# reuk/parallel-reverb-raytracer

Hardware: AMD Instinct MI355X
Metric: ray_bounces_per_sec (higher is better)
Workload: dtype f32; 1 GPU; cathedral stand-in (Sibenik unavailable offline), 75252 triangles, 100000 rays/GPU x 128 bounces x 8 bands, 2 cardioid speakers, 44100 Hz, trim_predelay, output_mode all, histogram mode exact; triangles=75252, rays_per_gpu=100000, reflections=128, histogram_mode=exact: the reference's serial float sum over all impulses, bit for bit

## Files before the change

include/rvb_capi.h:

```cpp
#ifndef RVB_CAPI_H
#define RVB_CAPI_H

#include <stdint.h>

#ifdef __cplusplus
extern "C" {
#endif

#define RVB_NUM_IMAGE_SOURCE 10
#define RVB_NUM_BANDS 8

enum {
    RVB_OK = 0,
    RVB_ERR_INVALID = 1,
    RVB_ERR_NO_DEVICE = 2,
    RVB_ERR_HIP = 3,
    RVB_ERR_STATE = 4,
    RVB_ERR_CAPACITY = 5
};

typedef struct { uint64_t surface, v0, v1, v2; } rvb_triangle;
typedef struct { float s[4]; } rvb_float3;
typedef struct { float specular[8]; float diffuse[8]; } rvb_surface;
typedef struct { float volume[8]; float position[4]; float time; float pad_[3]; } rvb_impulse;
// ... 17 lines not shown
int rvb_record_event(rvb_ctx * ctx, void * hip_event);
int rvb_device_info(rvb_ctx * ctx, char * arch, uint64_t arch_capacity, int * compute_units, uint64_t * hbm_bytes);
int rvb_device_index(rvb_ctx * ctx, int * device);

int rvb_set_scene(rvb_ctx * ctx,
                  const rvb_triangle * triangles, uint64_t ntriangles,
                  const rvb_float3 * vertices, uint64_t nvertices,
                  const rvb_surface * surfaces, uint64_t nsurfaces);
int rvb_share_scene(rvb_ctx * ctx, rvb_ctx * from);
int rvb_scene_info(rvb_ctx * ctx, uint64_t * nodes, uint64_t * kept_triangles, uint32_t * depth);

int rvb_set_directions(rvb_ctx * ctx, const rvb_float3 * directions, uint64_t nrays);
int rvb_set_directions_device(rvb_ctx * ctx, const void * d_directions, uint64_t nrays);
int rvb_set_concurrent_traces(rvb_ctx * ctx, uint32_t traces);
int rvb_set_path_lanes(rvb_ctx * ctx, uint32_t lanes);

int rvb_trace(rvb_ctx * ctx, const float mic[3], const float source[3],
              uint64_t nreflections, const float air_coefficient[8], uint64_t ray_offset);

int rvb_trace_pairs(rvb_ctx * ctx, const float * mics, const float * sources, uint64_t npairs,
                    uint64_t nreflections, const float air_coefficient[8], uint64_t ray_offset);

int rvb_trace_group(rvb_ctx ** ctxs, uint64_t count, const float * mics, const float * sources, uint64_t nreflections,
                    const float air_coefficient[8], const uint64_t * ray_offsets);
typedef struct { float direction[4]; float shape[8]; } rvb_source_pattern;
int rvb_set_source_pattern(rvb_ctx * ctx, const rvb_source_pattern * patterns, uint64_t npatterns);

int rvb_keep_paths(rvb_ctx * ctx, int keep);
int rvb_reshade(rvb_ctx * ctx, const rvb_surface * surfaces, uint64_t nsurfaces, const float air_coefficient[8]);

// ... 122 lines not shown
```

parallel-reverb-raytracer_amd/capi.py:

```python
import ctypes
import os

import numpy as np

from .dtypes import ATTENUATED, IMPULSE, SPEAKER, SURFACE, aligned_zeros

_HERE = os.path.dirname(os.path.abspath(__file__))
LIB_PATH = os.environ.get("RVB_LIB", os.path.join(_HERE, "librvb_hip.so"))

IMAGE_CANDIDATE = np.dtype([("ray", "<u8"), ("slot", "<u4"), ("index", "<u4"), ("impulse", IMPULSE)])
assert IMAGE_CANDIDATE.itemsize == 80

IR_DIFFUSE, IR_IMAGES, IR_ALL = 1, 2, 3
IR_FAST, IR_EXACT = 0, 1

SYMBOLS = [
    "rvb_create", "rvb_destroy", "rvb_last_error", "rvb_synchronize", "rvb_wait_for_event", "rvb_device_info",
    "rvb_set_scene", "rvb_share_scene", "rvb_scene_info", "rvb_set_directions", "rvb_set_directions_device", "rvb_set_concurrent_traces", "rvb_set_path_lanes", "rvb_trace", "rvb_trace_group",
    "rvb_trace_pairs", "rvb_ir_select_pair",
    "rvb_get_diffuse", "rvb_diffuse_device", "rvb_get_direct", "rvb_get_image_candidates", "rvb_merge_images",
    "rvb_attenuate_speaker", "rvb_attenuate_speaker_device", "rvb_attenuate_hrtf", "rvb_attenuate_hrtf_device", "rvb_flatten",
    "rvb_ir_configure_speakers", "rvb_ir_configure_hrtf", "rvb_ir_time_range", "rvb_ir_time_range_begin", "rvb_ir_bins", "rvb_ir_accumulate", "rvb_ir_accumulate_export", "rvb_ir_exact_prepare", "rvb_ir_exact_fold", "rvb_record_event",
    "rvb_ir_download", "rvb_last_timings", "rvb_debug_stamps", "rvb_executed_bounces",
    "rvb_device_alloc", "rvb_device_free", "rvb_copy_to_host", "rvb_copy_to_device", "rvb_fix_predelay_device", "rvb_flatten_device",
    "rvb_host_alloc", "rvb_host_free", "rvb_copy_to_pinned_host_async", "rvb_synchronize_exports",
    "rvb_multi_create", "rvb_multi_destroy", "rvb_multi_last_error", "rvb_multi_devices", "rvb_multi_context", "rvb_multi_used_rccl", "rvb_multi_set_chain_blocks", "rvb_multi_peer_links",
    "rvb_multi_set_scene", "rvb_multi_set_directions", "rvb_multi_trace", "rvb_multi_get_diffuse", "rvb_multi_get_images",
    "rvb_multi_ir_speakers", "rvb_multi_ir_hrtf",
    "rvb_device_index", "rvb_pipeline_create", "rvb_pipeline_destroy", "rvb_pipeline_last_error", "rvb_pipeline_configure_speakers",
    "rvb_pipeline_configure_hrtf", "rvb_pipeline_submit", "rvb_pipeline_submit_oriented", "rvb_pipeline_pending", "rvb_pipeline_next",
    "rvb_pipeline_create_lanes",
    "rvb_set_source_pattern", "rvb_multi_set_source_pattern", "rvb_pipeline_set_source_pattern", "rvb_pipeline_submit_directed",
    "rvb_keep_paths", "rvb_reshade",
# ... 174 lines not shown
        handles = (ctypes.c_void_p * n)(*[c.handle for c in contexts])
        m = np.ascontiguousarray(np.asarray(mics, dtype=np.float32).reshape(n, 3))
        s = np.ascontiguousarray(np.asarray(sources, dtype=np.float32).reshape(n, 3))
        offs = (ctypes.c_uint64 * n)(*[int(o) for o in (ray_offsets if ray_offsets is not None else [0] * n)])
        contexts[0]._check(contexts[0].lib.rvb_trace_group(handles, _u64(n), _ptr(m), _ptr(s), _u64(nreflections), _f8(air), offs))
        for c in contexts:
            c.nreflections = int(nreflections)
            c.npairs = 1

    def set_concurrent_traces(self, traces):
        self._check(self.lib.rvb_set_concurrent_traces(self.handle, ctypes.c_uint32(int(traces))))

    def set_path_lanes(self, lanes):
        self._check(self.lib.rvb_set_path_lanes(self.handle, ctypes.c_uint32(int(lanes))))

    def set_source_pattern(self, direction, shape=None):
        if direction is None or shape is None:
            self._check(self.lib.rvb_set_source_pattern(self.handle, None, _u64(0)))
            return
        pats = make_source_patterns(direction, shape)
        self._check(self.lib.rvb_set_source_pattern(self.handle, pats, _u64(len(pats))))

    def keep_paths(self, on):
        self._check(self.lib.rvb_keep_paths(self.handle, ctypes.c_int(1 if on else 0)))

    def reshade(self, surfaces, air):
        table, count = surface_table(surfaces)
        self._check(self.lib.rvb_reshade(self.handle, _ptr(table), _u64(count), _f8(air)))

    def trace(self, mic, source, nreflections, air, ray_offset=0):
# ... 383 lines not shown
```

parallel-reverb-raytracer_amd/csrc/bvh.h:

```cpp
#pragma once

#include <stdint.h>
#include <string>
#include <vector>

#include "../../include/rvb_capi.h"

#define RVB_BVH_EMPTY 0xFFFFFFFFu
#define RVB_BVH_LEAF 0x80000000u
#define RVB_BVH_NODE_SHIFT 6
#ifndef RVB_BVH_MAX_LEAF
#define RVB_BVH_MAX_LEAF 4
#endif
#define RVB_BVH_STACK 64

struct BvhChild {
    uint16_t lox, hix, loy, hiy, loz, hiz;
    uint32_t ref;
};
struct BvhNode { BvhChild c[4]; };

struct BvhTri {
    float v0[3];
    float e0[3];
    float e1[3];
    uint32_t index;
    uint32_t surface;
    uint32_t pad;
};

struct TriCorners { float v[9]; float pad[3]; };

struct TriShade { float n[3]; uint32_t surface; uint32_t skip_ref; float skip_a; float skip_b; uint32_t group; };

struct BuiltScene {
    std::vector<BvhNode> nodes;
    std::vector<BvhTri> tris;
    std::vector<TriShade> shade;
    std::vector<TriCorners> corners;
    std::vector<uint32_t> leafpos;
    uint32_t depth = 0;
    uint32_t stack_need = 0;
    float pad = 0.0f;
    float bounds_lo[3] = {0, 0, 0}, bounds_hi[3] = {0, 0, 0};
};

std::string rvb_build_scene(const rvb_triangle * triangles, uint64_t ntriangles,
                            const rvb_float3 * vertices, uint64_t nvertices,
                            uint64_t nsurfaces, BuiltScene & out);
```

parallel-reverb-raytracer_amd/csrc/bvh_build.hip:

```cpp
#include "bvh.h"
#include "rvb_math.h"

#include <algorithm>
#include <cmath>
#include <cstdlib>
#include <cstring>
#include <limits>
#include <queue>
#include <tuple>

namespace {

struct Box {
    float lo[3], hi[3];
    void reset()
    {
        for (int a = 0; a < 3; ++a) { lo[a] = std::numeric_limits<float>::infinity(); hi[a] = -lo[a]; }
    }
    void grow(const float p[3])
    {
        for (int a = 0; a < 3; ++a) { lo[a] = std::min(lo[a], p[a]); hi[a] = std::max(hi[a], p[a]); }
    }
    void grow(const Box & b)
    {
// ... 360 lines not shown
        TriShade & sk = out.shade[t.index];
        sk.group = gid[t.index];
        if (sk.skip_ref == RVB_BVH_EMPTY) continue;
        const PlaneGroup & pg = pl.groups[gid[t.index]];
        const TriGeo & g = pl.geo[t.index];
        const double A = 6.0 * pg.delta + pg.g + 32.0 * eps * g.kappa * g.L + 1.74 * eps * (double) maxabs;
        const double B = 16.0 * eps * g.kappa + 4.0 * eps;
        const double C = 2.0 * pg.theta + pg.d + 8.0 * eps;
        const double a = std::max(0.01, C + A * (1.0 + 1e-4) / EPS), b = B * (1.0 + 1e-4) / EPS;
        sk.skip_a = std::nextafterf((float) a, 2.0f);
        sk.skip_b = std::nextafterf((float) b, 2.0f);
        if (!(a < 1.0)) sk.skip_ref = RVB_BVH_EMPTY;
    }
}

}

std::string rvb_build_scene(const rvb_triangle * triangles, uint64_t ntriangles,
                            const rvb_float3 * vertices, uint64_t nvertices,
                            uint64_t nsurfaces, BuiltScene & out)
{
    if (ntriangles >= (1ull << 24))
        return "too many triangles (limit 2^24: triangle byte offsets are formed with a 24-bit multiply, node references are 31-bit byte offsets)";
    out = BuiltScene();
    out.shade.resize(ntriangles);
    out.corners.resize(ntriangles);

    float maxabs = 0.0f;
    Box scene;
    scene.reset();
// ... 181 lines not shown
    for (size_t i = out.nodes.size(); i-- > 0;) {
        uint32_t nchild = 0, deepest = 0;
        for (int k = 0; k < 4; ++k) {
            uint32_t c = out.nodes[i].c[k].ref;
            if (c == RVB_BVH_EMPTY)
                continue;
            ++nchild;
            if (!(c & RVB_BVH_LEAF))
                deepest = std::max(deepest, need[c >> RVB_BVH_NODE_SHIFT]);
        }
        need[i] = (nchild ? nchild - 1 : 0) + deepest;
    }
    out.stack_need = need[0] + 1;
    if (out.stack_need <= RVB_BVH_STACK) {
        assign_skips(out, planes, maxabs);
        return "";
    }
    }
    return "BVH needs a deeper traversal stack than " + std::to_string(RVB_BVH_STACK) + " entries";
}
```

parallel-reverb-raytracer_amd/csrc/context.hip:

```cpp
#include "ctx.h"

#include <cstring>

static thread_local std::string g_create_error;

int fail(rvb_ctx * ctx, int code, const std::string & what)
{
    if (ctx) ctx->error = what; else g_create_error = what;
    return code;
}

extern "C" {

int rvb_create(rvb_ctx ** out, int device, unsigned flags)
{
    (void) flags;
    if (!out)
        return fail(nullptr, RVB_ERR_INVALID, "rvb_create: out is NULL");
    *out = nullptr;
    int count = 0;
    hipError_t e = hipGetDeviceCount(&count);
    if (e != hipSuccess || count <= 0)
        return fail(nullptr, RVB_ERR_NO_DEVICE,
                    std::string("rvb_create: no HIP device (") + (e != hipSuccess ? hipGetErrorString(e) : "count 0") +
// ... 104 lines not shown
        ctx->store = std::make_shared<SceneStore>();
        ctx->store->device = ctx->device;
    }
    SceneStore & st = *ctx->store;
    auto upload = [&](DevBuf & b, const void * src, size_t bytes) -> hipError_t {
        hipError_t e = b.ensure(bytes);
        if (e != hipSuccess || bytes == 0) return e;
        return hipMemcpy(b.p, src, bytes, hipMemcpyHostToDevice);
    };
    RVB_HIP(fail, ctx, upload(st.nodes, built.nodes.data(), built.nodes.size() * sizeof(BvhNode)));
    RVB_HIP(fail, ctx, upload(st.tris, built.tris.data(), built.tris.size() * sizeof(BvhTri)));
    for (size_t i = 0; i < built.shade.size() && i < built.leafpos.size(); ++i) built.shade[i].group = built.leafpos[i];
    RVB_HIP(fail, ctx, upload(st.shade, built.shade.data(), built.shade.size() * sizeof(TriShade)));
    RVB_HIP(fail, ctx, upload(st.corners, built.corners.data(), built.corners.size() * sizeof(TriCorners)));
    RVB_HIP(fail, ctx, upload(st.surfaces, surfaces, nsurfaces * sizeof(rvb_surface)));
    ctx->scene.nodes = st.nodes.as<const BvhNode>();
    ctx->scene.tris = st.tris.as<const BvhTri>();
    ctx->scene.shade = st.shade.as<const TriShade>();
    ctx->scene.corners = st.corners.as<const TriCorners>();
    ctx->scene.surfaces = st.surfaces.as<const rvb_surface>();
    ctx->scene.ntris = (uint32_t) built.tris.size();
    ctx->scene.cull_abs = built.pad;
    ctx->scene.cull_rel = 1e-4f;
    ctx->nnodes = built.nodes.size();
    ctx->kept = built.tris.size();
    ctx->depth = built.depth;
    ctx->stack_need = built.stack_need;
    ctx->nsurfaces = nsurfaces;
    ctx->have_scene = true;
    return RVB_OK;
// ... 2 lines not shown
int rvb_share_scene(rvb_ctx * ctx, rvb_ctx * from)
{
    if (!ctx || !from) return RVB_ERR_INVALID;
    if (ctx == from) return RVB_OK;
    if (!from->have_scene || !from->store) return fail(ctx, RVB_ERR_STATE, "rvb_share_scene: the other context holds no scene");
    if (from->device != ctx->device) return fail(ctx, RVB_ERR_INVALID, "rvb_share_scene: the contexts are on different devices (a scene is shared within one GPU's memory)");
    RVB_BIND(ctx);
    RVB_HIP(fail, ctx, hipStreamSynchronize(ctx->stream));
    ctx->store = from->store;
    ctx->scene = from->scene;
    ctx->nnodes = from->nnodes;
    ctx->kept = from->kept;
    ctx->depth = from->depth;
    ctx->stack_need = from->stack_need;
    ctx->nsurfaces = from->nsurfaces;
    ctx->have_scene = true;
    ctx->traced = false;
    return RVB_OK;
}

int rvb_scene_info(rvb_ctx * ctx, uint64_t * nodes, uint64_t * kept_triangles, uint32_t * depth)
{
    if (!ctx) return RVB_ERR_INVALID;
    if (!ctx->have_scene) return fail(ctx, RVB_ERR_STATE, "rvb_scene_info: no scene");
    if (nodes) *nodes = ctx->nnodes;
    if (kept_triangles) *kept_triangles = ctx->kept;
    if (depth) *depth = ctx->depth;
    return RVB_OK;
}

// ... 30 lines not shown
}

int rvb_set_concurrent_traces(rvb_ctx * ctx, uint32_t traces)
{
    if (!ctx) return RVB_ERR_INVALID;
    if (traces == 0 || traces > (1u << 20)) return fail(ctx, RVB_ERR_INVALID, "rvb_set_concurrent_traces: 1 .. 2^20");
    ctx->concurrent_traces = traces;
    return RVB_OK;
}

int rvb_set_path_lanes(rvb_ctx * ctx, uint32_t lanes)
{
    if (!ctx) return RVB_ERR_INVALID;
    if (lanes != 0 && lanes != 1 && lanes != 2 && lanes != 4) return fail(ctx, RVB_ERR_INVALID, "rvb_set_path_lanes: 0 (automatic), 1, 2 or 4");
    ctx->path_lanes = lanes;
    return RVB_OK;
}

int rvb_last_timings(rvb_ctx * ctx, char * names, uint64_t names_capacity, float * ms, uint64_t ms_capacity, uint64_t * count)
{
    if (!ctx || !count) return RVB_ERR_INVALID;
    RVB_BIND(ctx);
    RVB_HIP(fail, ctx, hipStreamSynchronize(ctx->stream));
    std::string joined;
    uint64_t n = 0;
    for (const Timing & t : ctx->timings) {
        float v = 0.0f;
        RVB_HIP(fail, ctx, hipEventElapsedTime(&v, t.start, t.stop));
        if (ms && n < ms_capacity) ms[n] = v;
        if (!joined.empty()) joined += ';';
// ... 36 lines not shown
```

parallel-reverb-raytracer_amd/csrc/ctx.h:

```cpp
#pragma once

#include "../../include/rvb_capi.h"
#include "hip_owned.h"
#include "kernels.h"

#include <cmath>
#include <cstddef>
#include <memory>
#include <string>
#include <vector>

#pragma GCC visibility push(hidden)

struct SceneStore {
    int device = 0;
    DevBuf nodes, tris, shade, corners, surfaces;
    ~SceneStore() { (void) hipSetDevice(device); }
};

struct SmallBlock {
    uint32_t candidate_count;
    uint32_t pad0_;
    unsigned long long executed;
    uint32_t range[2];
    uint32_t max_time_bits;
    uint32_t pad1_;
    uint32_t trace_range[2];
    uint32_t image_item_count;
    uint32_t pad2_[5];
    rvb_impulse direct;
};
// ... 13 lines not shown
    Event export_ready;
    Event path_done, side_done;
    Event prep_done, group_done;
    std::string error;
    std::string arch;
    int compute_units = 0;
    uint64_t hbm_bytes = 0;

    bool have_scene = false;
    std::shared_ptr<SceneStore> store;
    SceneDev scene;
    uint64_t nnodes = 0, kept = 0;
    uint32_t depth = 0;
    uint32_t stack_need = RVB_BVH_STACK;
    uint64_t nsurfaces = 0;

    DevBuf directions_own;
    const float4 * directions = nullptr;
    uint64_t nrays = 0;
    uint32_t concurrent_traces = 1;
    uint32_t path_lanes = 0;
    bool range_pending = false;
    int hrtf_table_ears = 0;
    bool traced = false;
    uint64_t nreflections = 0;
    float mic[3] = {0, 0, 0};
    uint64_t npairs = 1, traced_rays = 0, ir_pair = 0;
    std::vector<float> pair_mics_host;
    DevBuf pair_geom, pair_direct, pair_range;
    PinnedBuf pair_stage;
// ... 111 lines not shown
```

parallel-reverb-raytracer_amd/csrc/kernels.h:

```cpp
#pragma once

#include <hip/hip_runtime.h>
#include <stdint.h>

#include "../../include/rvb_capi.h"
#include "bvh.h"

struct SceneDev {
    const BvhNode * nodes = nullptr;
    const BvhTri * tris = nullptr;
    const TriShade * shade = nullptr;
    const TriCorners * corners = nullptr;
    const rvb_surface * surfaces = nullptr;
    uint32_t ntris = 0;
    float cull_abs = 0.0f;
    float cull_rel = 0.0f;
    unsigned long long * stamps = nullptr;
};

struct ImageItem { uint32_t ray, index; };
struct TraceArgs {
    SceneDev scene;
    const float4 * directions;
    rvb_impulse * impulses;
// ... 12 lines not shown
    uint32_t * time_range;
    uint64_t nrays;
    uint32_t nreflections;
    uint32_t stack_entries;
    uint32_t lds_surfaces;
    uint32_t path_lanes;
    uint32_t npairs;
    uint32_t rays_per_pair;
    const float4 * pair_mics;
    const float4 * pair_sources;
    uint64_t ray_offset;
    float mic[3];
    float source[3];
    float air[8];
    float * image_dist;
};

void rvb_launch_path(const TraceArgs & a, hipStream_t s);
uint32_t rvb_lds_surfaces(uint32_t stack_entries, uint64_t nsurfaces);
uint32_t rvb_path_lanes_for(uint64_t nrays, uint32_t concurrent);
#define RVB_MAX_GROUP 4
void rvb_launch_path_group(const TraceArgs * traces, uint32_t count, hipStream_t s);
uint32_t rvb_shadow_lanes();
void rvb_launch_images(const TraceArgs & a, hipStream_t s);
void rvb_launch_shadow(const TraceArgs & a, hipStream_t s);
struct SourcePatternDev { float direction[4]; float shape[8]; };
SourcePatternDev rvb_source_pattern_device_form(const rvb_source_pattern & p);
void rvb_launch_source_pattern(const TraceArgs & a, const SourcePatternDev * patterns, uint32_t npatterns, hipStream_t s);
void rvb_launch_path_keep(const TraceArgs & a, float4 * kept, hipStream_t s);
uint32_t rvb_reshade_lds_surfaces(uint64_t nsurfaces);
void rvb_launch_reshade(const TraceArgs & a, const float4 * kept, hipStream_t s);
void rvb_launch_reshade_images(const TraceArgs & a, hipStream_t s);
size_t rvb_group_records_temp_bytes(uint64_t n);
hipError_t rvb_group_records(void * temp, size_t temp_bytes, const uint32_t * keys, uint32_t * keys_scratch, uint32_t * order,
                             uint64_t n, uint32_t first_record, int begin_bit, int end_bit, hipStream_t s);
hipError_t rvb_group_records16(void * temp, size_t temp_bytes, const uint16_t * keys, uint16_t * keys_scratch, uint32_t * order,
                               uint64_t n, uint32_t first_record, int begin_bit, int end_bit, hipStream_t s);

#define RVB_HRTF_ROWS (360 * 180 + 1)
struct AttenuationModel {
// ... 45 lines not shown
```

parallel-reverb-raytracer_amd/csrc/shadow_kernels.hip:

```cpp
#include "traversal.h"

#include <algorithm>
#include <cstdlib>

namespace {

template <bool SURF_LDS>
struct ShadowJob {
    const TraceArgs & a;
    uint32_t c;
    uint64_t g, stride, total;
    v3 mic;
    float airA, airB;
    float4 * rec;
    float4 mine;
    v3 p;
    float diff, new_dist, mag;
    uint32_t surface;
    float tmin, tmax_seen;
    uint32_t pair;
    lds_float4_ptr surf_lds;
    uint32_t skip;

    __device__ __forceinline__ uint32_t skip_ref() const { return skip; }
// ... 112 lines not shown
            const float4 m4 = a.pair_mics[tag - 1u];
            mic = mk3(m4.x, m4.y, m4.z);
            pair = tag - 1u;
        }
        const float new_dist = dpp_f<QP_PAIR_HI>(aux.x), threshold = dpp_f<QP_PAIR_HI>(aux.y);
        const float4 * shade = reinterpret_cast<const float4 *>(a.scene.shade + dpp_u<QP_PAIR_HI>(__float_as_uint(aux.z)));
        const float4 sh = shade[0];
        const uint32_t skip_ref = __float_as_uint(shade[1].x);
        const uint32_t surface = __float_as_uint(sh.w);
        const v3 p = mk3(dpp_f<QP_PAIR_LO>(aux.x), dpp_f<QP_PAIR_LO>(aux.y), dpp_f<QP_PAIR_LO>(aux.z));
        const float diff = dpp_f<QP_PAIR_LO>(aux.w);
        const v3 b2p = mic - p;
        const float mag = length3(b2p);
        const v3 dir = normalize3(b2p);
        const uint32_t skip = fabsf(dot3(mk3(sh.x, sh.y, sh.z), dir)) > threshold ? skip_ref : RVB_BVH_EMPTY;
        const bool visible = !traverse_pair_any(a.scene, p, dir, mag, stack, skip);
        const float dist = visible ? new_dist + mag : 0.0f;
        float4 o = make_float4(0, 0, 0, 0);
        if (visible) {
            const float4 dc = surface_row<SURF_LDS>(a, surf_lds, surface, 2 + h);
            o.x = band_product(vol.x, air_attenuation(dist, air0) * 1.0f, dc.x, diff);
            o.y = band_product(vol.y, air_attenuation(dist, air1) * 1.0f, dc.y, diff);
            o.z = band_product(vol.z, air_attenuation(dist, air2) * 1.0f, dc.z, diff);
            o.w = band_product(vol.w, air_attenuation(dist, air3) * 1.0f, dc.w, diff);
        }
        const float t = seconds_per_meter() * dist;
        store_stream(rec + h, o);
        store_stream(rec + h + 2, h == 0 ? make_float4(p.x, p.y, p.z, 0.0f) : make_float4(t, 0.0f, 0.0f, 0.0f));
        uint32_t nonzero = (o.x != 0.0f || o.y != 0.0f || o.z != 0.0f || o.w != 0.0f) ? 1u : 0u;
        nonzero |= dpp_u<QP_SWAP1>(nonzero);
        if (nonzero) {
// ... 114 lines not shown
            o_hi.z = band_product(vol_hi.z, air_attenuation(dist, a.air[6]) * 1.0f, d_hi.z, diff);
            o_hi.w = band_product(vol_hi.w, air_attenuation(dist, a.air[7]) * 1.0f, d_hi.w, diff);
        }
        const float t = seconds_per_meter() * dist;
        store_stream(rec + 0, o_lo);
        store_stream(rec + 1, o_hi);
        store_stream(rec + 2, make_float4(p.x, p.y, p.z, 0.0f));
        store_stream(rec + 3, make_float4(t, 0.0f, 0.0f, 0.0f));
        const bool nonzero = o_lo.x != 0.0f || o_lo.y != 0.0f || o_lo.z != 0.0f || o_lo.w != 0.0f
                          || o_hi.x != 0.0f || o_hi.y != 0.0f || o_hi.z != 0.0f || o_hi.w != 0.0f;
        note_time(a, nonzero, true, pair, t, tmin, tmax_seen);
    }
    time_range_of_wave(a, tmin, tmax_seen);
}

}

uint32_t rvb_shadow_lanes()
{
    static const int lanes = getenv("RVB_SHADOW_LANES") ? atoi(getenv("RVB_SHADOW_LANES")) : 2;
    return lanes == 4 ? 4u : (lanes == 1 ? 1u : 2u);
}

void rvb_launch_shadow(const TraceArgs & a, hipStream_t s)
{
    const uint64_t total = a.nrays * (uint64_t) a.nreflections;
    if (total == 0) return;
    static const char * const per_cu_env = getenv("RVB_SHADOW_WG_PER_CU");
    static const uint64_t per_cu_set = per_cu_env ? strtoull(per_cu_env, nullptr, 10) : 0;
    const uint32_t lanes = rvb_shadow_lanes();
// ... 10 lines not shown
```

parallel-reverb-raytracer_amd/csrc/trace.hip:

```cpp
#include "ctx.h"

#include <algorithm>
#include <cstdlib>
#include <cstring>
#include <map>

namespace {

struct TracePlan {
    TraceArgs a;
    uint64_t npairs = 1, nrays = 0, nreflections = 0;
    int key_bits = 1;
};

int upload_source_patterns(rvb_ctx * ctx)
{
    if (ctx->source_dirty && !ctx->source_patterns.empty()) {
        const size_t bytes = ctx->source_patterns.size() * sizeof(SourcePatternDev);
        if (bytes > ctx->source_stage.cap || bytes > ctx->source_dev.cap) {
            if (ctx->source_dev.p) RVB_HIP(fail, ctx, hipStreamSynchronize(ctx->stream));
            RVB_HIP(fail, ctx, ctx->source_stage.ensure(bytes));
            RVB_HIP(fail, ctx, ctx->source_dev.ensure(bytes));
        }
        if (!ctx->source_stage_free) RVB_HIP(fail, ctx, hipEventCreateWithFlags(&ctx->source_stage_free.h, hipEventDisableTiming));
// ... 68 lines not shown
    a.impulses = ctx->impulses.as<rvb_impulse>();
    a.early = ctx->early.as<uint32_t>();
    a.candidates = ctx->candidates.as<rvb_image_candidate>();
    a.candidate_count = &small->candidate_count;
    a.image_items = reinterpret_cast<ImageItem *>(ctx->image_items.p);
    a.image_state = ctx->image_items.as<uint32_t>() + ((size_t) nrays * 9 + npairs) * 2;
    a.image_item_count = &small->image_item_count;
    a.direct = &small->direct;
    a.npairs = (uint32_t) npairs;
    a.rays_per_pair = (uint32_t) ctx->nrays;
    a.pair_mics = nullptr;
    a.pair_sources = nullptr;
    a.executed = &small->executed;
    a.time_range = small->trace_range;
    a.image_dist = ctx->keep_paths ? ctx->kept_image_dist.as<float>() : nullptr;
    if (npairs > 1) {
        const size_t geom_floats = 8 * npairs, init_words = 2 * npairs;
        const size_t stage_bytes = geom_floats * sizeof(float) + init_words * sizeof(uint32_t);
        if (stage_bytes > ctx->pair_stage.cap) {
            if (ctx->pair_stage.p) RVB_HIP(fail, ctx, hipStreamSynchronize(ctx->stream));
            RVB_HIP(fail, ctx, ctx->pair_stage.ensure(stage_bytes));
        }
        if (!ctx->pair_stage_free) RVB_HIP(fail, ctx, hipEventCreateWithFlags(&ctx->pair_stage_free.h, hipEventDisableTiming));
        else RVB_HIP(fail, ctx, hipEventSynchronize(ctx->pair_stage_free));
        float * geom = ctx->pair_stage.as<float>();
        uint32_t * init = reinterpret_cast<uint32_t *>(geom + geom_floats);
        std::memset(geom, 0, geom_floats * sizeof(float));
        for (uint64_t p = 0; p < npairs; ++p)
            for (int i = 0; i < 3; ++i) { geom[4 * p + i] = mics[3 * p + i]; geom[4 * (npairs + p) + i] = sources[3 * p + i]; }
        for (uint64_t p = 0; p < npairs; ++p) { init[2 * p] = 0xFFFFFFFFu; init[2 * p + 1] = 0u; }
// ... 60 lines not shown
    TraceArgs & a = plan.a;
    const uint64_t npairs = plan.npairs, nrays = plan.nrays, nreflections = plan.nreflections;
    const int key_bits = plan.key_bits;
    static const int group_bits = getenv("RVB_SHADOW_SORT_BITS") ? atoi(getenv("RVB_SHADOW_SORT_BITS")) : 16;
    RVB_HIP(fail, ctx, hipEventRecord(ctx->path_done, ctx->stream));
    RVB_HIP(fail, ctx, hipStreamWaitEvent(ctx->side_stream, ctx->path_done, 0));
    ctx->begin_timing("image_kernel", ctx->side_stream);
    a.scene.stamps = nullptr;
    rvb_launch_images(a, ctx->side_stream);
    ctx->end_timing(ctx->side_stream);
    RVB_HIP(fail, ctx, hipEventRecord(ctx->side_done, ctx->side_stream));
    a.scene.stamps = ctx->stamps.as<unsigned long long>() + 16;
    if (ctx->keep_paths) {
        ctx->begin_timing("path_keep_kernel");
        rvb_launch_path_keep(a, ctx->kept_paths.as<float4>(), ctx->stream);
        ctx->end_timing();
        RVB_HIP(fail, ctx, hipGetLastError());
    }
    if (a.sort_keys || a.sort_keys16) {
        ctx->begin_timing("record_sort_kernels");
        a.sort_order = ctx->sort_order.as<uint32_t>();
        RVB_HIP(fail, ctx, hipGetLastError());
        const uint64_t per_pair = ctx->nrays * nreflections;
        for (uint64_t p = 0; p < npairs; ++p) {
            if (a.sort_keys16) {
                const int end = std::min(16, key_bits);
                RVB_HIP(fail, ctx, rvb_group_records16(ctx->group_temp.p, ctx->group_temp.cap, a.sort_keys16 + p * per_pair,
                                                       ctx->sort_scratch.as<uint16_t>() + p * per_pair, a.sort_order + p * per_pair, per_pair,
                                                       (uint32_t) (p * per_pair), std::max(0, end - group_bits), end, ctx->stream));
            } else if (own_sort_enabled()) {
// ... 350 lines not shown
```

parallel-reverb-raytracer_amd/csrc/traversal.h:

```cpp
#pragma once

#include "kernels.h"
#include "quad.h"
#include "rvb_math.h"

#ifndef RVB_CYCLE_LEAF_NUM
#define RVB_CYCLE_LEAF_NUM 3
#define RVB_CYCLE_LEAF_DEN 1
#endif
#ifndef RVB_CYCLE_DONE_NUM
#define RVB_CYCLE_DONE_NUM 4
#define RVB_CYCLE_DONE_DEN 1
#endif
#ifndef RVB_PAIR_WAVES
#define RVB_PAIR_WAVES 6
#endif
#ifndef RVB_SHADOW_PAIR_WAVES
#define RVB_SHADOW_PAIR_WAVES 5
#endif
#ifndef RVB_SHADOW_WAVES
#define RVB_SHADOW_WAVES 8
#endif
#ifndef RVB_LANE_WAVES
#define RVB_LANE_WAVES 4
// ... 534 lines not shown
            atomicAdd(sc.stamps + 9, t_b - t_loop);
            atomicAdd(sc.stamps + 10, 1ull);
            atomicAdd(sc.stamps + 11, r_end - r_loop);
        }
    }
#endif
#undef RESET_QUERY_PAIRS
#undef RVB_PAIR_POP
#undef RVB_PAIR_EMPTY
#undef ref
#undef sp
#undef RVB_PAIR_LIMIT
}

__device__ __forceinline__ bool traverse_pair_any(const SceneDev & sc, const v3 o, const v3 d, const float tmax,
                                                  uint32_t * __restrict__ stack, const uint32_t skip)
{
    const uint32_t h = threadIdx.x & 1u;
    const uint32_t c0 = 2u * h;
    const uint32_t bit0 = 1u << c0, bit1 = 2u << c0, lt0 = bit0 - 1u, lt1 = bit1 - 1u;
    const char * node_base = reinterpret_cast<const char *>(sc.nodes);
    const char * tri_base = reinterpret_cast<const char *>(sc.tris);
    const uint32_t child_off = 32u * h;
    const float neg_cull = -sc.cull_abs;
    const float limit = fmaf(tmax, 1.0f + sc.cull_rel, sc.cull_abs);
    const float ix = clamp_inv(d.x), iy = clamp_inv(d.y), iz = clamp_inv(d.z);
    const float oix = o.x * ix, oiy = o.y * iy, oiz = o.z * iz;
    uint32_t sp = 0, ref = 0;
    for (;;) {
        while (!(ref & RVB_BVH_LEAF)) {
            const uint4 * np = reinterpret_cast<const uint4 *>(node_base + (ref | child_off));
            const uint4 n0 = np[0], n1 = np[1];
            float tn0, tn1;
            const bool ok0 = slab(n0, ix, iy, iz, oix, oiy, oiz, limit, neg_cull, skip, tn0);
            const bool ok1 = slab(n1, ix, iy, iz, oix, oiy, oiz, limit, neg_cull, skip, tn1);
            uint32_t okmask = (ok0 ? bit0 : 0u) | (ok1 ? bit1 : 0u);
            okmask |= dpp_u<QP_SWAP1>(okmask);
            if (okmask == 0u) {
                if (sp > 0) { --sp; ref = stack[sp * PAIRS_PER_BLOCK]; } else ref = NONE;
                continue;
            }
            const uint32_t rest = okmask & (okmask - 1u);
            const uint32_t winner_bit = okmask ^ rest;
// ... 144 lines not shown
```

Before: 3.125 billion ray-bounces/s.

## Seed shadow-ray traversal with precomputed per-leaf BVH entry lists

Adds per-leaf entry lists: for each BVH leaf, a kernel run once per trace computes a short list (up to 7) of BVH subtrees whose bounds can meet the hull between that leaf and the mic. Shadow rays then start traversal from this list instead of the root, so fewer top-level nodes are visited per visibility test. The cost is an extra kernel per trace, a 32-byte row per triangle of device memory, and a conservative double-precision hull test that must stay correct to keep visibility exact. It is enabled by default when there is one pair and two shadow lanes.

```diff
diff --git a/include/rvb_capi.h b/include/rvb_capi.h
--- a/include/rvb_capi.h
+++ b/include/rvb_capi.h
@@ -55,6 +55,8 @@
 int rvb_set_directions_device(rvb_ctx * ctx, const void * d_directions, uint64_t nrays);
 int rvb_set_concurrent_traces(rvb_ctx * ctx, uint32_t traces);
 int rvb_set_path_lanes(rvb_ctx * ctx, uint32_t lanes);
+int rvb_set_shadow_entry_lists(rvb_ctx * ctx, int on);
+int rvb_set_shadow_entry_limit(rvb_ctx * ctx, uint32_t longest);
 
 int rvb_trace(rvb_ctx * ctx, const float mic[3], const float source[3],
               uint64_t nreflections, const float air_coefficient[8], uint64_t ray_offset);
diff --git a/parallel-reverb-raytracer_amd/capi.py b/parallel-reverb-raytracer_amd/capi.py
--- a/parallel-reverb-raytracer_amd/capi.py
+++ b/parallel-reverb-raytracer_amd/capi.py
@@ -16,7 +16,7 @@
 
 SYMBOLS = [
     "rvb_create", "rvb_destroy", "rvb_last_error", "rvb_synchronize", "rvb_wait_for_event", "rvb_device_info",
-    "rvb_set_scene", "rvb_share_scene", "rvb_scene_info", "rvb_set_directions", "rvb_set_directions_device", "rvb_set_concurrent_traces", "rvb_set_path_lanes", "rvb_trace", "rvb_trace_group",
+    "rvb_set_scene", "rvb_share_scene", "rvb_scene_info", "rvb_set_directions", "rvb_set_directions_device", "rvb_set_concurrent_traces", "rvb_set_path_lanes", "rvb_set_shadow_entry_lists", "rvb_set_shadow_entry_limit", "rvb_trace", "rvb_trace_group",
     "rvb_trace_pairs", "rvb_ir_select_pair",
     "rvb_get_diffuse", "rvb_diffuse_device", "rvb_get_direct", "rvb_get_image_candidates", "rvb_merge_images",
     "rvb_attenuate_speaker", "rvb_attenuate_speaker_device", "rvb_attenuate_hrtf", "rvb_attenuate_hrtf_device", "rvb_flatten",
@@ -221,6 +221,11 @@
     def set_path_lanes(self, lanes):
         self._check(self.lib.rvb_set_path_lanes(self.handle, ctypes.c_uint32(int(lanes))))
 
+    def set_shadow_entry_lists(self, on, longest=None):
+        self._check(self.lib.rvb_set_shadow_entry_lists(self.handle, ctypes.c_int(1 if on else 0)))
+        if longest is not None:
+            self._check(self.lib.rvb_set_shadow_entry_limit(self.handle, ctypes.c_uint32(int(longest))))
+
     def set_source_pattern(self, direction, shape=None):
         if direction is None or shape is None:
             self._check(self.lib.rvb_set_source_pattern(self.handle, None, _u64(0)))
diff --git a/parallel-reverb-raytracer_amd/csrc/bvh.h b/parallel-reverb-raytracer_amd/csrc/bvh.h
--- a/parallel-reverb-raytracer_amd/csrc/bvh.h
+++ b/parallel-reverb-raytracer_amd/csrc/bvh.h
@@ -33,6 +33,12 @@
 
 struct TriShade { float n[3]; uint32_t surface; uint32_t skip_ref; float skip_a; float skip_b; uint32_t group; };
 
+struct LeafEntry {
+    float lo[3], hi[3];
+    uint32_t ref;
+    uint32_t skip;
+};
+
 struct BuiltScene {
     std::vector<BvhNode> nodes;
     std::vector<BvhTri> tris;
@@ -41,6 +47,7 @@
     std::vector<uint32_t> leafpos;
     uint32_t depth = 0;
     uint32_t stack_need = 0;
+    std::vector<LeafEntry> leaves;
     float pad = 0.0f;
     float bounds_lo[3] = {0, 0, 0}, bounds_hi[3] = {0, 0, 0};
 };
diff --git a/parallel-reverb-raytracer_amd/csrc/bvh_build.hip b/parallel-reverb-raytracer_amd/csrc/bvh_build.hip
--- a/parallel-reverb-raytracer_amd/csrc/bvh_build.hip
+++ b/parallel-reverb-raytracer_amd/csrc/bvh_build.hip
@@ -1,4 +1,5 @@
 #include "bvh.h"
+#include "entry_lists.h"
 #include "rvb_math.h"
 
 #include <algorithm>
@@ -398,6 +399,48 @@
     }
 }
 
+void entry_leaves(BuiltScene & out, const std::vector<uint32_t> & need)
+{
+    out.leaves.clear();
+    std::vector<uint32_t> skip_refs;
+    for (const BvhTri & t : out.tris)
+        if (out.shade[t.index].skip_ref != RVB_BVH_EMPTY) skip_refs.push_back(out.shade[t.index].skip_ref);
+    std::sort(skip_refs.begin(), skip_refs.end());
+    uint32_t below = 0;
+    struct Item { uint32_t node, level; };
+    std::vector<Item> todo(1, Item{0u, 0u});
+    while (!todo.empty()) {
+        const Item it = todo.back();
+        todo.pop_back();
+        for (int k = 0; k < 4; ++k) {
+            const BvhChild & ch = out.nodes[it.node].c[k];
+            if (ch.ref == RVB_BVH_EMPTY) continue;
+            if (ch.ref & RVB_BVH_LEAF) {
+                LeafEntry e;
+                e.lo[0] = rvb_entry_half(ch.lox); e.lo[1] = rvb_entry_half(ch.loy); e.lo[2] = rvb_entry_half(ch.loz);
+                e.hi[0] = rvb_entry_half(ch.hix); e.hi[1] = rvb_entry_half(ch.hiy); e.hi[2] = rvb_entry_half(ch.hiz);
+                e.ref = ch.ref;
+                const uint32_t first = ch.ref & 0x0FFFFFFFu, count = ((ch.ref >> 28) & 7u) + 1u;
+                e.skip = out.shade[out.tris[first].index].skip_ref;
+                for (uint32_t j = 1; j < count; ++j)
+                    if (out.shade[out.tris[first + j].index].skip_ref != e.skip) e.skip = 0xFFFFFFFEu;
+                out.leaves.push_back(e);
+                continue;
+            }
+            const uint32_t child = ch.ref >> RVB_BVH_NODE_SHIFT;
+            if (it.level < RVB_ENTRY_CUT_MIN) {
+                const bool listed = it.level + 1u == RVB_ENTRY_CUT_MIN || std::binary_search(skip_refs.begin(), skip_refs.end(), ch.ref);
+                if (listed) below = std::max(below, need[child]);
+            }
+            todo.push_back(Item{child, it.level + 1u});
+        }
+    }
+    std::sort(out.leaves.begin(), out.leaves.end(), [](const LeafEntry & x, const LeafEntry & y) { return (x.ref & 0x0FFFFFFFu) < (y.ref & 0x0FFFFFFFu); });
+    const uint32_t with_lists = (RVB_ENTRY_K - 1) + below + 1;
+    if (with_lists > RVB_BVH_STACK) out.leaves.clear();
+    else out.stack_need = std::max(out.stack_need, with_lists);
+}
+
 }
 
 std::string rvb_build_scene(const rvb_triangle * triangles, uint64_t ntriangles,
@@ -609,6 +652,7 @@
     out.stack_need = need[0] + 1;
     if (out.stack_need <= RVB_BVH_STACK) {
         assign_skips(out, planes, maxabs);
+        entry_leaves(out, need);
         return "";
     }
     }
diff --git a/parallel-reverb-raytracer_amd/csrc/context.hip b/parallel-reverb-raytracer_amd/csrc/context.hip
--- a/parallel-reverb-raytracer_amd/csrc/context.hip
+++ b/parallel-reverb-raytracer_amd/csrc/context.hip
@@ -142,6 +142,10 @@
     RVB_HIP(fail, ctx, upload(st.shade, built.shade.data(), built.shade.size() * sizeof(TriShade)));
     RVB_HIP(fail, ctx, upload(st.corners, built.corners.data(), built.corners.size() * sizeof(TriCorners)));
     RVB_HIP(fail, ctx, upload(st.surfaces, surfaces, nsurfaces * sizeof(rvb_surface)));
+    RVB_HIP(fail, ctx, upload(st.leaves, built.leaves.data(), built.leaves.size() * sizeof(LeafEntry)));
+    RVB_HIP(fail, ctx, ctx->entry_rows.ensure(built.leaves.empty() ? 0 : built.tris.size() * 32));
+    ctx->leaf_entries = st.leaves.as<const LeafEntry>();
+    ctx->nleaves = (uint32_t) built.leaves.size();
     ctx->scene.nodes = st.nodes.as<const BvhNode>();
     ctx->scene.tris = st.tris.as<const BvhTri>();
     ctx->scene.shade = st.shade.as<const TriShade>();
@@ -174,6 +178,9 @@
     ctx->depth = from->depth;
     ctx->stack_need = from->stack_need;
     ctx->nsurfaces = from->nsurfaces;
+    RVB_HIP(fail, ctx, ctx->entry_rows.ensure(from->nleaves ? (size_t) from->kept * 32 : 0));
+    ctx->leaf_entries = from->leaf_entries;
+    ctx->nleaves = from->nleaves;
     ctx->have_scene = true;
     ctx->traced = false;
     return RVB_OK;
@@ -234,6 +241,21 @@
     if (!ctx) return RVB_ERR_INVALID;
     if (lanes != 0 && lanes != 1 && lanes != 2 && lanes != 4) return fail(ctx, RVB_ERR_INVALID, "rvb_set_path_lanes: 0 (automatic), 1, 2 or 4");
     ctx->path_lanes = lanes;
+    return RVB_OK;
+}
+
+int rvb_set_shadow_entry_lists(rvb_ctx * ctx, int on)
+{
+    if (!ctx) return RVB_ERR_INVALID;
+    ctx->entry_lists = on != 0;
+    return RVB_OK;
+}
+
+int rvb_set_shadow_entry_limit(rvb_ctx * ctx, uint32_t longest)
+{
+    if (!ctx) return RVB_ERR_INVALID;
+    if (longest == 0 || longest > 7) return fail(ctx, RVB_ERR_INVALID, "rvb_set_shadow_entry_limit: 1 .. 7");
+    ctx->entry_kmax = longest;
     return RVB_OK;
 }
 
diff --git a/parallel-reverb-raytracer_amd/csrc/ctx.h b/parallel-reverb-raytracer_amd/csrc/ctx.h
--- a/parallel-reverb-raytracer_amd/csrc/ctx.h
+++ b/parallel-reverb-raytracer_amd/csrc/ctx.h
@@ -15,6 +15,7 @@
 struct SceneStore {
     int device = 0;
     DevBuf nodes, tris, shade, corners, surfaces;
+    DevBuf leaves;
     ~SceneStore() { (void) hipSetDevice(device); }
 };
 
@@ -58,6 +59,11 @@
     uint32_t depth = 0;
     uint32_t stack_need = RVB_BVH_STACK;
     uint64_t nsurfaces = 0;
+    const LeafEntry * leaf_entries = nullptr;
+    uint32_t nleaves = 0;
+    bool entry_lists = true;
+    uint32_t entry_kmax = 7;
+    DevBuf entry_rows;
 
     DevBuf directions_own;
     const float4 * directions = nullptr;
diff --git a/parallel-reverb-raytracer_amd/csrc/entry_lists.h b/parallel-reverb-raytracer_amd/csrc/entry_lists.h
--- /dev/null
+++ b/parallel-reverb-raytracer_amd/csrc/entry_lists.h
@@ -0,0 +1,105 @@
+#pragma once
+
+#include <math.h>
+#include <stdint.h>
+#include <string.h>
+
+#include "bvh.h"
+
+#if defined(__HIPCC__)
+#include <hip/hip_runtime.h>
+#define RVB_ENTRY_HD __host__ __device__ inline
+#else
+#define RVB_ENTRY_HD inline
+#endif
+
+#define RVB_ENTRY_K 7
+#define RVB_ENTRY_CUT 4
+#define RVB_ENTRY_CUT_MIN 3
+#define RVB_ENTRY_CUT_MAX 6
+#define RVB_ENTRY_ROUNDING 4e-6
+
+struct EntryRow { uint32_t w[8]; };
+
+RVB_ENTRY_HD float rvb_entry_half(uint16_t b)
+{
+    return (float) __builtin_bit_cast(_Float16, b);
+}
+
+RVB_ENTRY_HD bool rvb_entry_hull_meets(const double blo[3], const double bhi[3], const double m[3], const double nlo[3], const double nhi[3])
+{
+    double s0 = 0.0, s1 = 1.0;
+    for (int a = 0; a < 3; ++a) {
+        const double a0 = m[a] - blo[a], b0 = nhi[a] - blo[a];
+        if (a0 > 0.0) { const double s = b0 / a0; if (s < s1) s1 = s; }
+        else if (a0 < 0.0) { const double s = b0 / a0; if (s > s0) s0 = s; }
+        else if (b0 < 0.0) return false;
+        const double a1 = m[a] - bhi[a], b1 = nlo[a] - bhi[a];
+        if (a1 > 0.0) { const double s = b1 / a1; if (s > s0) s0 = s; }
+        else if (a1 < 0.0) { const double s = b1 / a1; if (s < s1) s1 = s; }
+        else if (b1 > 0.0) return false;
+    }
+    return s0 - 1e-9 <= s1 + 1e-9;
+}
+
+RVB_ENTRY_HD uint32_t rvb_entry_row(const BvhNode * nodes, uint32_t depth, const LeafEntry & leaf, const float mic[3], float cull_abs, float cull_rel,
+                                    uint32_t kmax, uint32_t cut, EntryRow & row)
+{
+    for (int i = 1; i < 8; ++i) row.w[i] = RVB_BVH_EMPTY;
+    row.w[0] = 1u; row.w[1] = 0u;
+    if (cut < RVB_ENTRY_CUT_MIN || cut > RVB_ENTRY_CUT_MAX || kmax == 0u || kmax > RVB_ENTRY_K || leaf.skip == 0xFFFFFFFEu)
+        return 0u;
+    double blo[3], bhi[3], m[3], len2 = 0.0, big = 0.0;
+    for (int a = 0; a < 3; ++a) {
+        blo[a] = leaf.lo[a]; bhi[a] = leaf.hi[a]; m[a] = mic[a];
+        const double far = (m[a] - blo[a] > bhi[a] - m[a]) ? m[a] - blo[a] : bhi[a] - m[a];
+        len2 += far * far;
+        const double c0 = blo[a] < 0 ? -blo[a] : blo[a], c1 = bhi[a] < 0 ? -bhi[a] : bhi[a], c2 = m[a] < 0 ? -m[a] : m[a];
+        if (c0 > big) big = c0;
+        if (c1 > big) big = c1;
+        if (c2 > big) big = c2;
+    }
+    if (!(len2 == len2) || !(big < 1e30)) return 0u;
+    const double len = sqrt(len2) * (1.0 + 1e-12);
+    for (; cut >= RVB_ENTRY_CUT_MIN; --cut) {
+        if (depth <= cut) continue;
+        uint32_t list[RVB_ENTRY_K];
+        uint32_t n = 0;
+        bool fits = true;
+        uint32_t todo[16], todo_level[16], ntodo = 0;
+        todo[ntodo] = 0u; todo_level[ntodo++] = 0u;
+        while (ntodo && fits) {
+            const uint32_t ref = todo[--ntodo], level = todo_level[ntodo];
+            const BvhNode & node = nodes[ref >> RVB_BVH_NODE_SHIFT];
+            for (int k = 0; k < 4 && fits; ++k) {
+                const BvhChild & ch = node.c[k];
+                if (ch.ref == RVB_BVH_EMPTY) continue;
+                double nlo[3] = {rvb_entry_half(ch.lox), rvb_entry_half(ch.loy), rvb_entry_half(ch.loz)};
+                double nhi[3] = {rvb_entry_half(ch.hix), rvb_entry_half(ch.hiy), rvb_entry_half(ch.hiz)};
+                double nbig = big;
+                for (int a = 0; a < 3; ++a) {
+                    const double c0 = nlo[a] < 0 ? -nlo[a] : nlo[a], c1 = nhi[a] < 0 ? -nhi[a] : nhi[a];
+                    if (c0 < 1e30 && c0 > nbig) nbig = c0;
+                    if (c1 < 1e30 && c1 > nbig) nbig = c1;
+                }
+                const double widen = (double) cull_abs + (double) cull_rel * len + RVB_ENTRY_ROUNDING * (nbig + len);
+                for (int a = 0; a < 3; ++a) { nlo[a] -= widen; nhi[a] += widen; }
+                if (!rvb_entry_hull_meets(blo, bhi, m, nlo, nhi)) continue;
+                const bool is_skip = ch.ref == leaf.skip;
+                if ((ch.ref & RVB_BVH_LEAF) || is_skip || level + 1u >= cut) {
+                    if (n == kmax) { fits = false; break; }
+                    list[n++] = ch.ref;
+                    if (is_skip) { const uint32_t t = list[0]; list[0] = list[n - 1]; list[n - 1] = t; }
+                } else {
+                    todo[ntodo] = ch.ref; todo_level[ntodo++] = level + 1u;
+                }
+            }
+        }
+        if (!fits) continue;
+        row.w[0] = n ? n : 1u;
+        row.w[1] = RVB_BVH_EMPTY;
+        for (uint32_t i = 0; i < n; ++i) row.w[1 + i] = list[i];
+        return cut;
+    }
+    return 0u;
+}
diff --git a/parallel-reverb-raytracer_amd/csrc/kernels.h b/parallel-reverb-raytracer_amd/csrc/kernels.h
--- a/parallel-reverb-raytracer_amd/csrc/kernels.h
+++ b/parallel-reverb-raytracer_amd/csrc/kernels.h
@@ -50,6 +50,7 @@
     float source[3];
     float air[8];
     float * image_dist;
+    const uint4 * entry_rows;
 };
 
 void rvb_launch_path(const TraceArgs & a, hipStream_t s);
@@ -60,6 +61,8 @@
 uint32_t rvb_shadow_lanes();
 void rvb_launch_images(const TraceArgs & a, hipStream_t s);
 void rvb_launch_shadow(const TraceArgs & a, hipStream_t s);
+void rvb_launch_entry_rows(const SceneDev & scene, uint32_t depth, const LeafEntry * leaves, uint32_t nleaves, const float mic[3], uint32_t kmax,
+                           uint4 * rows, hipStream_t s);
 struct SourcePatternDev { float direction[4]; float shape[8]; };
 SourcePatternDev rvb_source_pattern_device_form(const rvb_source_pattern & p);
 void rvb_launch_source_pattern(const TraceArgs & a, const SourcePatternDev * patterns, uint32_t npatterns, hipStream_t s);
diff --git a/parallel-reverb-raytracer_amd/csrc/shadow_kernels.hip b/parallel-reverb-raytracer_amd/csrc/shadow_kernels.hip
--- a/parallel-reverb-raytracer_amd/csrc/shadow_kernels.hip
+++ b/parallel-reverb-raytracer_amd/csrc/shadow_kernels.hip
@@ -1,4 +1,5 @@
 #include "traversal.h"
+#include "entry_lists.h"
 
 #include <algorithm>
 #include <cstdlib>
@@ -150,7 +151,21 @@
         const float mag = length3(b2p);
         const v3 dir = normalize3(b2p);
         const uint32_t skip = fabsf(dot3(mk3(sh.x, sh.y, sh.z), dir)) > threshold ? skip_ref : RVB_BVH_EMPTY;
-        const bool visible = !traverse_pair_any(a.scene, p, dir, mag, stack, skip);
+        uint32_t ref = 0, sp = 0;
+        if (a.entry_rows) {
+            const uint4 e = a.entry_rows[2u * __float_as_uint(shade[1].w) + h];
+            if (h == 0) {
+                stack[0 * PAIRS_PER_BLOCK] = e.z; stack[1 * PAIRS_PER_BLOCK] = e.w;
+            } else {
+                stack[2 * PAIRS_PER_BLOCK] = e.x; stack[3 * PAIRS_PER_BLOCK] = e.y; stack[4 * PAIRS_PER_BLOCK] = e.z; stack[5 * PAIRS_PER_BLOCK] = e.w;
+            }
+            sp = dpp_u<QP_PAIR_LO>(e.x) - 1u;
+            ref = dpp_u<QP_PAIR_LO>(e.y);
+            if (ref == skip) {
+                if (sp > 0) { --sp; ref = stack[sp * PAIRS_PER_BLOCK]; } else ref = NONE;
+            }
+        }
+        const bool visible = !traverse_pair_any(a.scene, p, dir, mag, stack, skip, ref, sp);
         const float dist = visible ? new_dist + mag : 0.0f;
         float4 o = make_float4(0, 0, 0, 0);
         if (visible) {
@@ -295,6 +310,32 @@
     time_range_of_wave(a, tmin, tmax_seen);
 }
 
+__global__ __launch_bounds__(WAVE) void entry_rows_kernel(const BvhNode * nodes, uint32_t depth, const LeafEntry * leaves, uint32_t nleaves,
+                                                          float mx, float my, float mz, float cull_abs, float cull_rel, uint32_t kmax, uint32_t cut,
+                                                          uint32_t ntris, uint4 * rows)
+{
+    const uint32_t i = blockIdx.x * WAVE + threadIdx.x;
+    if (i >= nleaves) return;
+    const LeafEntry leaf = leaves[i];
+    const float mic[3] = {mx, my, mz};
+    EntryRow row;
+    rvb_entry_row(nodes, depth, leaf, mic, cull_abs, cull_rel, kmax, cut, row);
+    const uint32_t first = leaf.ref & 0x0FFFFFFFu, count = ((leaf.ref >> 28) & 7u) + 1u;
+    for (uint32_t j = 0; j < count && first + j < ntris; ++j) {
+        rows[2u * (first + j)] = make_uint4(row.w[0], row.w[1], row.w[2], row.w[3]);
+        rows[2u * (first + j) + 1u] = make_uint4(row.w[4], row.w[5], row.w[6], row.w[7]);
+    }
+}
+
+}
+
+void rvb_launch_entry_rows(const SceneDev & scene, uint32_t depth, const LeafEntry * leaves, uint32_t nleaves, const float mic[3], uint32_t kmax,
+                           uint4 * rows, hipStream_t s)
+{
+    if (nleaves == 0) return;
+    static const uint32_t cut = getenv("RVB_SHADOW_ENTRY_CUT") ? std::min<uint32_t>(RVB_ENTRY_CUT_MAX, std::max<uint32_t>(RVB_ENTRY_CUT_MIN, (uint32_t) atoi(getenv("RVB_SHADOW_ENTRY_CUT")))) : RVB_ENTRY_CUT;
+    hipLaunchKernelGGL(entry_rows_kernel, dim3((nleaves + WAVE - 1) / WAVE), dim3(WAVE), 0, s, scene.nodes, depth, leaves, nleaves,
+                       mic[0], mic[1], mic[2], scene.cull_abs, scene.cull_rel, kmax, cut, scene.ntris, rows);
 }
 
 uint32_t rvb_shadow_lanes()
diff --git a/parallel-reverb-raytracer_amd/csrc/trace.hip b/parallel-reverb-raytracer_amd/csrc/trace.hip
--- a/parallel-reverb-raytracer_amd/csrc/trace.hip
+++ b/parallel-reverb-raytracer_amd/csrc/trace.hip
@@ -106,6 +106,8 @@
     a.executed = &small->executed;
     a.time_range = small->trace_range;
     a.image_dist = ctx->keep_paths ? ctx->kept_image_dist.as<float>() : nullptr;
+    static const bool lists_env_off = getenv("RVB_SHADOW_ENTRY_LISTS") && getenv("RVB_SHADOW_ENTRY_LISTS")[0] == '0';
+    a.entry_rows = (ctx->entry_lists && !lists_env_off && npairs == 1 && ctx->nleaves && ctx->entry_rows.p && rvb_shadow_lanes() == 2) ? ctx->entry_rows.as<uint4>() : nullptr;
     if (npairs > 1) {
         const size_t geom_floats = 8 * npairs, init_words = 2 * npairs;
         const size_t stage_bytes = geom_floats * sizeof(float) + init_words * sizeof(uint32_t);
@@ -196,6 +198,12 @@
     if (ctx->keep_paths) {
         ctx->begin_timing("path_keep_kernel");
         rvb_launch_path_keep(a, ctx->kept_paths.as<float4>(), ctx->stream);
+        ctx->end_timing();
+        RVB_HIP(fail, ctx, hipGetLastError());
+    }
+    if (a.entry_rows) {
+        ctx->begin_timing("entry_rows_kernel");
+        rvb_launch_entry_rows(a.scene, ctx->depth, ctx->leaf_entries, ctx->nleaves, a.mic, ctx->entry_kmax, ctx->entry_rows.as<uint4>(), ctx->stream);
         ctx->end_timing();
         RVB_HIP(fail, ctx, hipGetLastError());
     }
diff --git a/parallel-reverb-raytracer_amd/csrc/traversal.h b/parallel-reverb-raytracer_amd/csrc/traversal.h
--- a/parallel-reverb-raytracer_amd/csrc/traversal.h
+++ b/parallel-reverb-raytracer_amd/csrc/traversal.h
@@ -572,7 +572,7 @@
 }
 
 __device__ __forceinline__ bool traverse_pair_any(const SceneDev & sc, const v3 o, const v3 d, const float tmax,
-                                                  uint32_t * __restrict__ stack, const uint32_t skip)
+                                                  uint32_t * __restrict__ stack, const uint32_t skip, uint32_t ref = 0, uint32_t sp = 0)
 {
     const uint32_t h = threadIdx.x & 1u;
     const uint32_t c0 = 2u * h;
@@ -584,7 +584,6 @@
     const float limit = fmaf(tmax, 1.0f + sc.cull_rel, sc.cull_abs);
     const float ix = clamp_inv(d.x), iy = clamp_inv(d.y), iz = clamp_inv(d.z);
     const float oix = o.x * ix, oiy = o.y * iy, oiz = o.z * iz;
-    uint32_t sp = 0, ref = 0;
     for (;;) {
         while (!(ref & RVB_BVH_LEAF)) {
             const uint4 * np = reinterpret_cast<const uint4 *>(node_base + (ref | child_off));
```

Result: no change. 3.102 billion ray-bounces/s (-0.7%).
